# adelowo/cap

Hardware: AMD Instinct MI355X
Metric: verified JWTs/sec (RS256-2048, ES256) at 1/2/4/8 MI355X vs all-core Go CPU (higher is better)
Workload: dtype u32 (28-bit limbs, 64-bit v_mad_u64_u32 accumulators); 1 GPU; ES256 P-256 JWKS with 4 kids, 1M tokens batch-verified per MI355X (BASELINE configs[1]); kids=4, p256_key_comb_w=26, parallelism=independent shards x1

## Files before the change

### cap_amd/csrc/jg_runtime.cpp

```cpp
#include <pthread.h>
#include <hip/hip_runtime.h>
#include <sched.h>

#include <algorithm>
#include <array>
#include <atomic>
#include <chrono>
#include <condition_variable>
#include <cstddef>
#include <cstdio>
#include <cstdlib>
#include <cstring>
#include <deque>
#include <functional>
#include <map>
#include <set>
#include <memory>
#include <mutex>
#include <shared_mutex>
#include <string>
#include <thread>
#include <unordered_map>
#include <vector>

// ... 38 lines not shown
    const char* e = std::getenv("CAPJWT_RELEASE_GTABLES");
    return e && std::atoi(e) != 0;
  }();
  return on;
}

double ms_since(std::chrono::steady_clock::time_point t) {
  return std::chrono::duration<double, std::milli>(std::chrono::steady_clock::now() - t).count();
}

bool load_trace() {
  static const bool on = std::getenv("CAPJWT_LOAD_TRACE") != nullptr;
  return on;
}
struct PhaseClock {
  std::chrono::steady_clock::time_point t = std::chrono::steady_clock::now();
  void lap(const char* what) {
    if (!load_trace()) return;
    std::fprintf(stderr, "[capjwt load] %-28s %8.2f ms\n", what, ms_since(t));
    t = std::chrono::steady_clock::now();
  }
};

bool zc_env_enabled() {
  const char* e = std::getenv("CAPJWT_ZC");
  return e && std::atoi(e) != 0;
}
size_t zc_env_max_jobs() {
  const char* e = std::getenv("CAPJWT_ZC_MAX");
  const long long v = e ? std::atoll(e) : 0;
  return v >= 64 ? (size_t)v : (size_t)2 << 20;
}

size_t chunk_jobs() {
  static const size_t n = [] {
    if (const char* e = std::getenv("CAPJWT_CHUNK")) {
      const long v = std::atol(e);
      if (v >= 64) return (size_t)v;
    }
    return (size_t)65536;
  }();
  return n;
}

uint64_t default_table_budget() {
  static const uint64_t b = [] {
    if (const char* e = std::getenv("CAPJWT_TABLE_BUDGET_GB")) {
      const double v = std::atof(e);
      if (v >= 0) return (uint64_t)(v * (double)(1ull << 30));
    }
    return (uint64_t)32 << 30;
  }();
  return b;
}

std::vector<size_t> chunk_cuts(size_t lo, size_t hi, size_t C, size_t first = 4096, bool tail_chunk = true) {
  std::vector<size_t> cut{lo};
  for (size_t ramp = std::min<size_t>(C, first); cut.back() < hi; ramp = std::min(C, 2 * ramp))
    cut.push_back(std::min(hi, cut.back() + ramp));
  const size_t tail = C / 4;
  if (tail_chunk && cut.size() > 2 && tail >= 1024 && cut.back() - cut[cut.size() - 2] > tail)
    cut.insert(cut.end() - 1, cut.back() - tail);
  else if (!tail_chunk && cut.size() > 2 && cut.back() - cut[cut.size() - 2] < C / 8)
    cut.erase(cut.end() - 2);
  return cut;
}

int cls_rows_sig(int c, int l4) {
  switch (c) {
    case CLS_RSA2K: case CLS_RSA3K: return rsa_sig_rows(c);
    case CLS_RSA4K: return rsa_sig_rows_l(l4);
    case CLS_P256: case CLS_P384: case CLS_P521: return EC_S_ROW + 17;
    case CLS_ED25519: return 16;
    default: return 0;
  }
}
int cls_rows_scratch(int c, int l4) {
  switch (c) {
    case CLS_RSA2K: case CLS_RSA3K: return 2 * rsa_limbs(c) + rsa_sig_rows(c);
    case CLS_RSA4K: return 2 * l4 + rsa_sig_rows_l(l4);
    case CLS_P256: case CLS_P384: case CLS_P521: return ec_digit_rows(c) + 2 * ec_limbs(c);
    case CLS_ED25519: return 4 * ED_L;
    default: return 0;
  }
}
constexpr double CLS_COST[NCLS] = {0.01, 4.2, 9.0, 15.5, 1.0, 3.4, 6.6, 1.1};

inline size_t grow_size(size_t n, size_t cap) {
  const size_t want = std::max(n, cap + cap / 2);
  return (want + (size_t(2) << 20) - 1) & ~((size_t(2) << 20) - 1);
}

std::atomic<int> g_grows{0};

struct Grow {
  void* p = nullptr;
  size_t cap = 0;
  void* get(size_t n) {
    if (n == 0) n = 16;
    if (n > cap) {
      if (p) (void)hipFree(p);
      p = nullptr;
      const size_t c = grow_size(n, cap);
      cap = 0;
      g_grows.fetch_add(1, std::memory_order_relaxed);
      HIPCHK(hipMalloc(&p, c));
// ... 331 lines not shown
  bool zc = false;
  bool small_ec = true;
  std::atomic<uint64_t>* small_launches = nullptr;
};

class Helper {
 public:
  explicit Helper(int device) : th_([this, device] { loop(device); }) {}
  ~Helper() {
    {
      std::lock_guard<std::mutex> g(m_);
      stop_ = true;
    }
    cv_.notify_all();
    th_.join();
  }
  void run(std::function<void()> f) {
    std::lock_guard<std::mutex> g(m_);
    job_ = std::move(f);
    busy_ = true;
    cv_.notify_all();
  }
  void wait() {
    std::unique_lock<std::mutex> lk(m_);
    cv_.wait(lk, [&] { return !busy_; });
  }

 private:
  void loop(int device) {
    pthread_setname_np(pthread_self(), "capjwt-plan");
    (void)hipSetDevice(device);
    std::unique_lock<std::mutex> lk(m_);
    while (true) {
      cv_.wait(lk, [&] { return stop_ || job_; });
      if (!job_) break;
      auto f = std::move(job_);
      job_ = nullptr;
      lk.unlock();
      f();
      lk.lock();
      busy_ = false;
      cv_.notify_all();
    }
  }
  std::mutex m_;
  std::condition_variable cv_;
  std::function<void()> job_;
  bool busy_ = false, stop_ = false;
  std::thread th_;
};

struct Device {
  int id = 0;
  Lane lane0;
  Lane lane1;
  hipStream_t kstream = nullptr;
  hipStream_t ustream = nullptr;
  hipStream_t clstream = nullptr;
  std::mutex cl_mu;
  Grow cl_arena, cl_jobs, cl_out, cl_expect;
  uint32_t* gtab[NCLS] = {};
  uint32_t* btab = nullptr;
  std::shared_ptr<SharedTable> tab_ref[NCLS];
  std::mutex mu;
  hipStream_t copy = nullptr;
  Lane lanes[NLANE];
  Slot slots[NSLOT + NZSLOT];
  int next_slot = 0, next_lane = 0, next_zslot = 0;
  double gload[3] = {0, 0, 0};
  int next_res = 0;
  std::thread worker, completer;
  std::unique_ptr<Helper> planner;
  std::mutex qmu;
  std::condition_variable qcv;
  std::deque<Item> q;
  bool stop = false;
  std::mutex cmu;
  std::condition_variable ccv, scv;
  std::deque<Slot*> cq;
  bool cstop = false;
};

}

struct jg_batch {
  jg_ctx* ctx = nullptr;
  Device* dev = nullptr;
  Lane* lane = nullptr;
  std::unique_ptr<Bufs> own;
  Bufs* b = nullptr;
  Plan plan;
  size_t arena_len = 0;
  size_t dslot = 0;
  uint64_t epoch = 0;
  KeyStateP ks_run;
  bool timing = true;
  std::vector<std::string> mark_names;
  std::vector<hipEvent_t> mark_events;
  size_t marks_used = 0;
  std::vector<std::string> tnames;
  std::vector<float> tms;
  ~jg_batch() {
    for (auto e : mark_events) (void)hipEventDestroy(e);
  }
};

// ... 249 lines not shown
    P.sig_rows = std::max(P.sig_rows, cls_rows_sig(c, P.rsa4k_limbs));
    P.scratch_rows = std::max(P.scratch_rows, cls_rows_scratch(c, P.rsa4k_limbs));
    if (c <= CLS_RSA4K) {
      P.pss_off[c] = P.pss_tokens;
      P.pss_tokens += P.ranges[c].end - P.ranges[c].begin;
    }
  }
}

inline std::pair<int64_t, int64_t> pad_range(const PlanScratch& X, size_t b, const Plan& P, size_t RB) {
  if (P.npad == WAVE && X.start[RB] == 0 && b == RB) {
    int64_t any = 0;
    for (int64_t t : X.total) any += t;
    if (any == 0) return {0, WAVE};
  }
  return {X.start[b] + X.total[b], X.start[b] + (X.total[b] + WAVE - 1) / WAVE * WAVE};
}

void plan_fill_host(const KeyState& K, const jg_tok* toks, size_t ntok, const Plan& P, PlanScratch& X, JobDev* jobs,
                    int32_t* perm) {
  const size_t nk = K.keys.size(), NB = nk + 1, RB = nk;
  for (size_t b = 0; b < NB; ++b) {
    const auto r = pad_range(X, b, P, RB);
    const JobDev pad{0, 0, 0, job_pack(b == RB ? 0u : (uint32_t)b, JOB_PAD, 0)};
    for (int64_t p = r.first; p < r.second; ++p) {
      jobs[p] = pad;
      perm[p] = -1;
    }
  }
  std::vector<int64_t> cur = X.start;
  for (size_t i = 0; i < ntok; ++i) {
    const jg_tok& tk = toks[i];
    const int c = X.tcls[i];
    const int64_t p = cur[c == CLS_REJECT ? RB : tk.key_idx]++;
    jobs[p] = JobDev{(uint32_t)tk.off, tk.sig_in_len, (uint32_t)(tk.off + tk.sig_rel_off),
                     job_pack(c == CLS_REJECT ? 0u : tk.key_idx, tk.alg, tk.sig_b64_len)};
    perm[p] = (int32_t)i;
  }
}

void size_scratch(Bufs* B, const Plan& P, size_t arena_bytes) {
  const int64_t npad = P.npad;
  const size_t ntok = std::max<size_t>((size_t)P.ntok, 1);
  B->arena.get(arena_bytes + ARENA_SLACK);
  B->sigw.get(sizeof(uint32_t) * P.sig_rows * npad);
  B->dig.get(sizeof(uint32_t) * DIG_ROWS * npad);
  B->status.get(npad);
  B->siglen.get(sizeof(uint16_t) * npad);
  B->vpad.get(npad);
  B->verdict.get(ntok);
  B->rows.get(sizeof(uint32_t) * (size_t)P.scratch_rows * npad);
  B->pss.get((size_t)std::max<int64_t>(P.pss_tokens, 1) * 2048);
  B->exc.get(sizeof(int32_t) * npad);
  B->exc_cnt.get(sizeof(uint32_t) * NCLS);
}

void upload(Bufs* B, hipStream_t s, const Plan& P, const uint8_t* arena, size_t arena_bytes, const JobDev* jobs,
            const int32_t* perm) {
  size_scratch(B, P, arena_bytes);
  B->jobs.get(sizeof(JobDev) * P.npad);
  B->perm.get(sizeof(int32_t) * P.npad);
  uint8_t* da = (uint8_t*)B->arena.p;
  if (arena_bytes && arena) HIPCHK(hipMemcpyAsync(da, arena, arena_bytes, hipMemcpyHostToDevice, s));
  HIPCHK(hipMemsetAsync(da + arena_bytes, 0, ARENA_SLACK, s));
  HIPCHK(hipMemcpyAsync(B->jobs.p, jobs, sizeof(JobDev) * P.npad, hipMemcpyHostToDevice, s));
  HIPCHK(hipMemcpyAsync(B->perm.p, perm, sizeof(int32_t) * P.npad, hipMemcpyHostToDevice, s));
}

struct PlanBlock {
  size_t cur_off, pad_off, zc_off, toks_off, bytes;
  PlanBlock(size_t nbuckets, size_t n) {
    cur_off = 0;
    pad_off = sizeof(uint64_t) * nbuckets;
    zc_off = pad_off + 2 * sizeof(int64_t) * nbuckets;
    toks_off = (zc_off + 3 * sizeof(uint64_t) * nbuckets + 63) & ~size_t(63);
    bytes = toks_off + sizeof(jg_tok) * std::max<size_t>(n, 1);
  }
};

void mark(jg_batch* b, const char* name) {
  if (!b || !b->timing) return;
  if (b->marks_used == b->mark_events.size()) {
    hipEvent_t e;
    HIPCHK(hipEventCreate(&e));
    b->mark_events.push_back(e);
    b->mark_names.emplace_back();
  }
  HIPCHK(hipEventRecord(b->mark_events[b->marks_used], b->lane->stream));
  b->mark_names[b->marks_used] = name;
  ++b->marks_used;
}

const char* cls_name(int c) {
  static const char* n[NCLS] = {"reject", "rsa2048", "rsa3072", "rsa4096", "p256", "p384", "p521", "ed25519"};
  return n[c];
}

struct MarkCtx {
  jg_batch* b;
  int cls;
};
thread_local MarkCtx g_mark_ctx;

void mark_cb(void* p, const char* kname) {
  MarkCtx* m = (MarkCtx*)p;
  mark(m->b, (std::string(cls_name(m->cls)) + "_" + kname).c_str());
}
// ... 108 lines not shown
  for (int oi = 0; oi < NCLS - 1; ++oi) {
    const int c = order[oi];
    const ClassRange r = P.ranges[c];
    if (r.end <= r.begin) continue;
    hipStream_t s = s0;
    if (conc) {
      s = L->cstream[c];
      HIPCHK(hipStreamWaitEvent(s, L->ev_start, 0));
    } else if (gf) {
      s = gf->cls[c];
      if (!feed) HIPCHK(hipStreamWaitEvent(s, gf->start, 0));
    }
    if (zc) {
      ZcGatherArgs za = gf->gather;
      za.begin = r.begin;
      za.end = r.end;
      launch_zc_gather(za, feed ? gf->feed : s);
      if (feed) {
        HIPCHK(hipEventRecord(gf->fed[c], gf->feed));
        HIPCHK(hipStreamWaitEvent(s, gf->fed[c], 0));
      }
    }
    pa.begin = r.begin;
    pa.end = r.end;
    pa.zrows = cls_rows_sig(c, P.rsa4k_limbs);
    pa.ec_words = (c >= CLS_P256 && c <= CLS_P521) ? ec_sig_words(c) : 0;
    launch_prep(c, P.hash_mask[c], pa, s);
    mark(marks, (std::string(cls_name(c)) + "_prep").c_str());
    if (c <= CLS_RSA4K) {
      RsaArgs ra{};
      ra.jobs = pa.jobs; ra.keys = pa.keys; ra.keyblob = pa.keyblob;
      ra.sigw = pa.sigw; ra.dig = pa.dig;
      const int Lm = c == CLS_RSA4K ? P.rsa4k_limbs : rsa_limbs(c);
      ra.xmw = rows;
      ra.xlr = rows + (size_t)Lm * np;
      ra.yw = rows + (size_t)2 * Lm * np;
      ra.status = pa.status; ra.siglen = pa.siglen; ra.verdict_pad = (uint8_t*)B->vpad.p;
      ra.pss_scratch = (uint8_t*)B->pss.p + P.pss_off[c] * 2048;
      ra.has_pss = P.pss_any[c];
      ra.layouts = c == CLS_RSA4K ? P.rsa4k_layouts : 1;
      ra.npad = np; ra.begin = r.begin; ra.end = r.end;
      launch_rsa(c, ra, s, marker(marks, c));
    } else if (c <= CLS_P521) {
      if (!d->gtab[c]) throw std::runtime_error("curve table missing");
      EcArgs ea{};
      ea.jobs = pa.jobs; ea.keys = pa.keys; ea.keyblob = pa.keyblob;
      ea.sigw = pa.sigw; ea.dig = pa.dig; ea.status = pa.status; ea.verdict_pad = (uint8_t*)B->vpad.p;
      ea.digs = rows;
      ea.u1w = rows + (size_t)ec_digit_rows(c) * np;
      ea.u2w = rows + (size_t)(ec_digit_rows(c) + ec_limbs(c)) * np;
      ea.gtab = d->gtab[c];
      ea.exc_list = (int32_t*)B->exc.p + r.begin;
      ea.exc_count = (uint32_t*)B->exc_cnt.p + c;
      ea.npad = np;
      ea.exc_reset = 1;
      ea.part = EC_FAST;
      width_runs(K, G, P, c, [&](int64_t b, int64_t e, int w) {
        ea.begin = b; ea.end = e; ea.wq = w;
        launch_ec(c, ea, s, marker(marks, c));
        ea.exc_reset = 0;
      });
      EcArgs x = ea;
      x.begin = r.begin;
      x.end = r.end;
      x.part = EC_EXACT;
      if (gf) exact_later.push_back({c, x});
      else launch_ec(c, x, s, marker(marks, c));
    } else {
      if (!d->btab) throw std::runtime_error("Ed25519 base table missing");
      EdArgs ea{};
      ea.jobs = pa.jobs; ea.keys = pa.keys; ea.keyblob = pa.keyblob;
      ea.sigw = pa.sigw; ea.dig = pa.dig; ea.status = pa.status; ea.siglen = pa.siglen;
      ea.verdict_pad = (uint8_t*)B->vpad.p;
      ea.xyz = rows;
      ea.btab = d->btab;
      ea.npad = np;
      width_runs(K, G, P, c, [&](int64_t b, int64_t e, int w) {
        ea.begin = b; ea.end = e; ea.wa = w;
        launch_ed(ea, s, marker(marks, c));
      });
    }
    if (s != s0) G.uses.record(s, conc ? "class stream" : "group lane", c);
    if (conc) {
      HIPCHK(hipEventRecord(L->ev_done[c], s));
      HIPCHK(hipStreamWaitEvent(s0, L->ev_done[c], 0));
    } else if (gf) {
      HIPCHK(hipEventRecord(gf->done[c], s));
      if (s != s0) HIPCHK(hipStreamWaitEvent(s0, gf->done[c], 0));
    }
  }
  for (const auto& [c, x] : exact_later) launch_ec(c, x, s0, Marker{});
  launch_scatter((const int32_t*)B->perm.p, (const uint8_t*)B->vpad.p,
                 verdict_dst ? verdict_dst : (uint8_t*)B->verdict.p, np, s0);
  mark(marks, "scatter");
  HIPCHK(hipGetLastError());
  G.uses.record(s0, gf ? "join lane" : "lane");
}

void collect_times(jg_batch* b) {
  b->tnames.clear();
  b->tms.clear();
  for (size_t i = 1; i < b->marks_used; ++i) {
    float ms = 0;
    if (hipEventElapsedTime(&ms, b->mark_events[i - 1], b->mark_events[i]) == hipSuccess) {
      b->tnames.push_back(b->mark_names[i]);
      b->tms.push_back(ms);
// ... 1189 lines not shown
    it.nchunks = it.cuts.size() - 1;
    t->pending += it.nchunks;
    items.push_back(std::move(it));
  }
  for (size_t k = 0, i = 0; k < nd && i < items.size(); ++k) {
    if (cut[k + 1] <= cut[k]) continue;
    Device* d = ctx->devs[k].get();
    Item& it = items[i++];
    if (it.nchunks == 1 && it.hi - it.lo <= SMALL_SUBMIT) {
      bool idle;
      {
        std::lock_guard<std::mutex> g(d->qmu);
        idle = d->q.empty();
      }
      if (idle) {
        process_item(d, k, it);
        continue;
      }
    }
    {
      std::lock_guard<std::mutex> g(d->qmu);
      d->q.push_back(std::move(it));
    }
    d->qcv.notify_one();
  }
  return t;
}

int wait_ticket(jg_ctx* ctx, const std::shared_ptr<Ticket>& t) {
  std::unique_lock<std::mutex> lk(t->m);
  t->cv.wait(lk, [&] { return t->pending == 0; });
  if (t->rc) ctx->set_err(t->err);
  return t->rc;
}

}

extern "C" {

jg_ctx* jg_create(const int* devices, int ndev) {
  try {
    auto ctx = std::make_unique<jg_ctx>();
    int count = 0;
    HIPCHK(hipGetDeviceCount(&count));
    if (count <= 0) throw std::runtime_error("no HIP device");
    std::vector<int> ids;
    if (!devices || ndev <= 0) ids.push_back(0);
    else ids.assign(devices, devices + ndev);
    for (int id : ids) {
      if (id < 0 || id >= count) throw std::runtime_error("bad device id " + std::to_string(id));
      auto d = std::make_unique<Device>();
      d->id = id;
      HIPCHK(hipSetDevice(id));
      HIPCHK(hipStreamCreateWithFlags(&d->copy, hipStreamNonBlocking));
      for (auto& l : d->lanes) l.create_main();
      d->lane0.create_main();
      d->lane1.create_main();
      d->lane0.create_fanout(RES_GROUP, RES_NGROUPS);
      d->lane1.create_fanout(RES_GROUP, RES_NGROUPS);
      for (auto& s : d->slots) {
        HIPCHK(hipEventCreateWithFlags(&s.done, pipe_trace() ? hipEventDefault : hipEventDisableTiming));
        HIPCHK(hipEventCreateWithFlags(&s.copied, hipEventDisableTiming));
        HIPCHK(hipEventCreate(&s.tr_a));
        HIPCHK(hipEventCreate(&s.tr_b));
        HIPCHK(hipEventCreate(&s.tr_c));
        HIPCHK(hipEventCreateWithFlags(&s.ev_planned, hipEventDisableTiming));
        for (auto& e : s.ev_cls) HIPCHK(hipEventCreateWithFlags(&e, hipEventDisableTiming));
        for (auto& e : s.ev_fed) HIPCHK(hipEventCreateWithFlags(&e, hipEventDisableTiming));
      }
      HIPCHK(hipStreamCreateWithFlags(&d->kstream, hipStreamNonBlocking));
      HIPCHK(hipStreamCreateWithFlags(&d->ustream, hipStreamNonBlocking));
      HIPCHK(hipStreamCreateWithFlags(&d->clstream, hipStreamNonBlocking));
      ctx->devs.push_back(std::move(d));
    }
    auto ks = std::make_shared<KeyState>();
    for (size_t i = 0; i < ctx->devs.size(); ++i) ks->dev.push_back(std::make_shared<DevGen>());
    ctx->ks = ks;
    jg_ctx* c = ctx.release();
    for (size_t i = 0; i < c->devs.size(); ++i) {
      c->devs[i]->planner = std::make_unique<Helper>(c->devs[i]->id);
      c->devs[i]->worker = std::thread(worker_loop, c->devs[i].get(), i);
      c->devs[i]->completer = std::thread(completer_loop, c->devs[i].get());
    }
    c->upgrader = std::thread(upgrade_loop, c);
    return c;
  } catch (const std::exception& e) {
    g_tls_err = e.what();
    return nullptr;
  }
}

void jg_destroy(jg_ctx* ctx) {
  if (!ctx) return;
  {
    std::lock_guard<std::mutex> g(ctx->up_mu);
    ctx->up_stop = true;
  }
  ctx->up_cv.notify_all();
  if (ctx->upgrader.joinable()) ctx->upgrader.join();
  for (auto& d : ctx->devs) {
    {
      std::lock_guard<std::mutex> g(d->qmu);
      d->stop = true;
    }
    d->qcv.notify_all();
    if (d->worker.joinable()) d->worker.join();
// ... 507 lines not shown
```

### cap_amd/csrc/kernels/ecdsa.hpp

```cpp
#pragma once
#include <hip/hip_runtime.h>
#include <cstdint>

#include "common.hpp"
#include "prep.hpp"

struct EcArgs {
  const jgk::JobDev* jobs;
  const jgk::DevKey* keys;
  const uint32_t* keyblob;
  const uint32_t* sigw;
  const uint32_t* dig;
  uint8_t* status;
  uint8_t* verdict_pad;
  uint32_t* digs;
  uint32_t* u1w;
  uint32_t* u2w;
  const uint32_t* gtab;
  int32_t* exc_list;
  uint32_t* exc_count;
  int64_t npad, begin, end;
  int32_t wq;
  int32_t exc_reset;
  int32_t part;
};
enum : int32_t { EC_ALL = 0, EC_FAST = 1, EC_EXACT = 2 };

constexpr int ec_limbs(int cls) { return cls == jgk::CLS_P256 ? 10 : cls == jgk::CLS_P384 ? 15 : 20; }
constexpr int ec_sig_words(int cls) { return cls == jgk::CLS_P256 ? 8 : cls == jgk::CLS_P384 ? 12 : 17; }
#ifndef JG_EC_PACK64
#define JG_EC_PACK64 1
#endif
constexpr bool ec_packed(int cls) { return JG_EC_PACK64 && cls == jgk::CLS_P256; }
constexpr int ec_stride(int cls) { return ec_packed(cls) ? 16 : (2 * ec_limbs(cls) + 3) & ~3; }
constexpr int ec_order_bits(int cls) { return cls == jgk::CLS_P256 ? 256 : cls == jgk::CLS_P384 ? 384 : 521; }
constexpr int ec_comb_w(int cls, bool gen) {
  return cls == jgk::CLS_P256 ? (gen ? 26 : 20) : cls == jgk::CLS_P384 ? (gen ? 24 : 16) : (gen ? 20 : 16);
}
constexpr int ec_windows_w(int cls, int w) { return (ec_order_bits(cls) + 2 + w - 1) / w; }
constexpr int ec_entries(int cls, bool gen) { return 1 << (ec_comb_w(cls, gen) - 1); }
constexpr int ec_windows(int cls, bool gen) { return ec_windows_w(cls, ec_comb_w(cls, gen)); }
constexpr int ec_digit_rows(int cls) { return ec_windows(cls, true) + ec_windows(cls, false); }
constexpr int ec_max_keys(int cls) { return 256; }
constexpr int64_t ec_table_words_w(int cls, int w) {
  return (int64_t)ec_windows_w(cls, w) * (1 << (w - 1)) * ec_stride(cls);
}
constexpr int64_t ec_table_words(int cls, bool gen) { return ec_table_words_w(cls, ec_comb_w(cls, gen)); }
constexpr int EC_P256_WQ[4] = {26, 24, 22, 20};
constexpr int EC_P384_WQ[4] = {24, 20, 18, 16};
constexpr int EC_P521_WQ[3] = {20, 18, 16};
constexpr bool ec_top_window_ok(int cls, int w) { return ec_order_bits(cls) - w * (ec_windows_w(cls, w) - 1) <= w - 2; }
static_assert(ec_top_window_ok(jgk::CLS_P256, 26) && ec_top_window_ok(jgk::CLS_P256, 24) &&
              ec_top_window_ok(jgk::CLS_P256, 22) && ec_top_window_ok(jgk::CLS_P256, 20) &&
              ec_top_window_ok(jgk::CLS_P384, 24) && ec_top_window_ok(jgk::CLS_P384, 20) &&
              ec_top_window_ok(jgk::CLS_P384, 18) && ec_top_window_ok(jgk::CLS_P384, 16) &&
              ec_top_window_ok(jgk::CLS_P521, 20) && ec_top_window_ok(jgk::CLS_P521, 18) &&
              ec_top_window_ok(jgk::CLS_P521, 16), "comb window count leaves no room for the top carry");

void launch_ec(int cls, const EcArgs& a, hipStream_t s, const jgk::Marker& mk);

constexpr int EC_SMALL_MAX = jgk::SMALL_MAX;
constexpr uint32_t EC_SMALL_IN_MAX = jgk::SMALL_IN_MAX;
struct EcSmallArgs {
  const uint8_t* arena;
  const jgk::DevKey* keys;
  const uint32_t* keyblob;
  const uint32_t* gtab;
  uint8_t* verdict;
  uint32_t n;
  jgk::JobDev jobs[EC_SMALL_MAX];
  uint16_t out[EC_SMALL_MAX];
};
void launch_ec_small(int cls, int wq, const EcSmallArgs& a, hipStream_t s);
void launch_ec_keyprep(int cls, jgk::DevKey* keys, uint32_t* blob, const int32_t* idx, int n, hipStream_t s);
void launch_ec_keytables(int cls, int wq, jgk::DevKey* keys, uint32_t* blob, const int32_t* tidx, int tn,
                         hipStream_t s, bool sliced = false);
void launch_ec_gtable(int cls, uint32_t* tab, hipStream_t s);
```

### cap_amd/csrc/kernels/ecdsa_impl.hpp

```cpp
#pragma once
#include <hip/hip_runtime.h>

#include <algorithm>
#include <cstdlib>
#include <type_traits>

#include "common.hpp"
#include "ecdsa.hpp"
#include "inv_shape.hpp"
#include "mp.hpp"
#include "tables.hpp"

using namespace jgk;

namespace {

template <int WQ_>
struct CurveP256W { using Fp = P256P; using Fn = P256N; using C = P256C; static constexpr int CLS = CLS_P256, WQ = WQ_; };
using CurveP256 = CurveP256W<20>;
template <int WQ_>
struct CurveP384W { using Fp = P384P; using Fn = P384N; using C = P384C; static constexpr int CLS = CLS_P384, WQ = WQ_; };
using CurveP384 = CurveP384W<16>;
template <int WQ_>
struct CurveP521W { using Fp = P521P; using Fn = P521N; using C = P521C; static constexpr int CLS = CLS_P521, WQ = WQ_; };
// ... 130 lines not shown
  for (int q = 0; q < EW; ++q) {
    const int src = hw - 1 - q;
    R.ew[q] = src >= 0 ? a.dig[(int64_t)(src < 0 ? 0 : src) * np + p] : 0u;
  }
}

template <class CV>
__device__ __forceinline__ void ec_scalar_re(const EcArgs& a, int64_t p, uint32_t* r, uint32_t* e) {
  using Fn = typename CV::Fn;
  constexpr int L = Fn::L;
  ScalarRaw2<CV> R;
  ec_scalar_load2<CV>(a, p, -1, R);
  mp::words_to_limbs<L, ScalarRaw<CV>::CW>(r, R.rw);
  mp::words_to_limbs<L, ScalarRaw<CV>::EW>(e, R.ew);
  mp::csub<Fn>(e);
}

template <class CV, int W, int NWIN>
__device__ __forceinline__ void store_digit_rows(const EcArgs& a, int64_t p, const uint32_t* u, int row0) {
  constexpr int L = CV::Fn::L;
  constexpr uint32_t DM = (1u << W) - 1u;
  int c = 0;
#pragma unroll
  for (int w = 0; w < NWIN; ++w) {
    const int bit = W * w, q = bit / MP_W, sh = bit % MP_W;
    uint32_t b = q < L ? (u[q] >> sh) : 0u;
    if (sh > MP_W - W && q + 1 < L) b |= u[q + 1] << (MP_W - sh);
    int v = (int)(b & DM) + c;
    c = v >= (1 << (W - 1));
    v -= c << W;
    a.digs[(int64_t)(row0 + w) * a.npad + p] = (uint32_t)v;
  }
}

#ifndef JG_EC_SCALAR_WPB
#define JG_EC_SCALAR_WPB 4
#endif
#ifndef JG_EC_SCALAR_PF
#define JG_EC_SCALAR_PF 0
#endif
constexpr int EC_SCALAR_WPB = JG_EC_SCALAR_WPB;
template <class CV, int WPB = EC_SCALAR_WPB>
#ifndef JG_EC_SCALAR_ATTR
#define JG_EC_SCALAR_ATTR
#endif
__global__ void __launch_bounds__(64 * WPB) JG_EC_SCALAR_ATTR k_ec_scalar_batch(EcArgs a, int B) {
  using Fn = typename CV::Fn;
  constexpr int L = Fn::L;
  const int64_t np = a.npad;
  const int64_t n = a.end - a.begin;
  const int64_t S = (n + B - 1) / B;
  const int64_t i = (int64_t)blockIdx.x * blockDim.x + threadIdx.x;
  if (a.exc_reset && i == 0) *a.exc_count = 0u;
  if (WPB == 1 && i >= S) return;
  uint32_t acc[L];
  mp::set_const<Fn>(acc, Fn::ONE);
  int nb = 0;
  constexpr int WG = ec_comb_w(CV::CLS, true), NG = ec_windows(CV::CLS, true);
  constexpr int WQ = CV::WQ, NQ = ec_windows_w(CV::CLS, CV::WQ);
#if JG_EC_SCALAR_PF
  {
    ScalarRaw<CV> cur, nxt;
    int64_t p = a.begin + i;
    bool have = B > 0 && i < S && p < a.end;
    if (have) ec_scalar_load<CV>(a, p, cur);
    for (int j = 0; have; ++j) {
      const int64_t pn = p + S;
      const bool more = j + 1 < B && pn < a.end;
      if (more) ec_scalar_load<CV>(a, pn, nxt);
      uint32_t r[L], s[L], e[L], sm[L];
      const bool ok = ec_scalar_finish<CV>(a, p, cur, r, s, e);
      if (!ok && job_live(cur.jb)) a.status[p] = ST_REJECT;
      mp::to_mont<Fn>(sm, s);
      mp::mul<Fn>(acc, acc, sm);
#pragma unroll
      for (int k = 0; k < L; ++k) {
        a.u1w[(int64_t)k * np + p] = acc[k];
        a.u2w[(int64_t)k * np + p] = sm[k];
      }
      ++nb;
      if (!more) break;
      cur = nxt;
      p = pn;
    }
  }
  uint32_t inv[L];
  mp::block_inv<Fn, WPB>(inv, acc);
  if (nb > 0) {
    ScalarRaw2<CV> cur, nxt;
    int64_t p = a.begin + i + (int64_t)(nb - 1) * S;
    ec_scalar_load2<CV>(a, p, nb > 1 ? p - S : -1, cur);
    for (int j = nb - 1; j >= 0; --j) {
      if (j > 0) ec_scalar_load2<CV>(a, p - S, j > 1 ? p - 2 * S : -1, nxt);
      uint32_t w[L], r[L], e[L], u1[L], u2[L];
      mp::mul<Fn>(w, inv, cur.cprev);
      mp::mul<Fn>(inv, inv, cur.sm);
      mp::words_to_limbs<L, ScalarRaw<CV>::CW>(r, cur.rw);
      mp::words_to_limbs<L, ScalarRaw<CV>::EW>(e, cur.ew);
      mp::csub<Fn>(e);
      mp::mul<Fn>(u1, e, w); mp::csub<Fn>(u1);
      mp::mul<Fn>(u2, r, w); mp::csub<Fn>(u2);
      store_digit_rows<CV, WG, NG>(a, p, u1, 0);
      store_digit_rows<CV, WQ, NQ>(a, p, u2, NG);
      if (j == 0) break;
      cur = nxt;
      p -= S;
// ... 198 lines not shown
  const int ad = d < 0 ? -d : d;
  const uint32_t* ent = tab + ((int64_t)w * NE + (ad - 1)) * STRIDE;
  uint32_t x2[L], y2[L];
  load_entry<CV>(ent, x2, y2);
  if (d < 0) mp::neg<Fp>(y2, y2);
  if (empty) {
    mp::copy<Fp>(X, x2);
    mp::copy<Fp>(Y, y2); mp::freduce<Fp>(Y);
    mp::set_const<Fp>(Z, Fp::ONE);
    empty = false;
  } else if constexpr (Z1ONE) {
    madd_z1<Fp>(X, Y, Z, x2, y2);
  } else {
    madd<Fp>(X, Y, Z, x2, y2);
  }
}

template <class CV>
__device__ __forceinline__ void load_raw(const uint32_t* __restrict__ ent, uint4* r) {
  const uint4* e4 = reinterpret_cast<const uint4*>(ent);
#pragma unroll
  for (int i = 0; i < 4; ++i) r[i] = e4[i];
}
template <class CV, bool Z1ONE = false>
__device__ __forceinline__ void add_raw(uint32_t* X, uint32_t* Y, uint32_t* Z, bool& empty, const uint4* r, int d) {
  using Fp = typename CV::Fp;
  constexpr int L = Fp::L;
  if (d == 0) return;
  const uint32_t wx[8] = {r[0].x, r[0].y, r[0].z, r[0].w, r[1].x, r[1].y, r[1].z, r[1].w};
  const uint32_t wy[8] = {r[2].x, r[2].y, r[2].z, r[2].w, r[3].x, r[3].y, r[3].z, r[3].w};
  uint32_t x2[L], y2[L];
  mp::words_to_limbs<L, 8>(x2, wx);
  mp::words_to_limbs<L, 8>(y2, wy);
  if (d < 0) mp::neg<Fp>(y2, y2);
  if (empty) {
    mp::copy<Fp>(X, x2);
    mp::copy<Fp>(Y, y2); mp::freduce<Fp>(Y);
    mp::set_const<Fp>(Z, Fp::ONE);
    empty = false;
  } else if constexpr (Z1ONE) {
    madd_z1<Fp>(X, Y, Z, x2, y2);
  } else {
    madd<Fp>(X, Y, Z, x2, y2);
  }
}
#ifndef JG_EC_POINT_PF
#define JG_EC_POINT_PF 0
#endif

#ifndef JG_EC_POINT_ATTR
#define JG_EC_POINT_ATTR
#endif
template <class CV>
__global__ void __launch_bounds__(64) JG_EC_POINT_ATTR k_ec_point(EcArgs a) {
  using Fp = typename CV::Fp;
  using Fn = typename CV::Fn;
  constexpr int L = Fp::L;
  constexpr int NG = ec_windows(CV::CLS, true), NQ = ec_windows_w(CV::CLS, CV::WQ);
  constexpr int NWIN = NG > NQ ? NG : NQ;
  const int64_t p = a.begin + (int64_t)blockIdx.x * WAVE + threadIdx.x;
  const int64_t np = a.npad;
  const JobDev jb = a.jobs[p];
  if (!job_live(jb)) return;
  if (a.status[p] != ST_OK) { a.verdict_pad[p] = 0; return; }
  const int kidx = __builtin_amdgcn_readfirstlane(job_key(jb));
  const uint32_t* __restrict__ qtab = key_table(a.keys[kidx]);
  const uint32_t* __restrict__ gtab = a.gtab;

  uint32_t X[L], Y[L], Z[L];
  bool empty = true;
#if JG_EC_POINT_PF
  if constexpr (ec_packed(CV::CLS) && NG == NQ) {
    constexpr int NS = 2 * NG, STRIDE = ec_stride(CV::CLS);
    constexpr int NEG = ec_entries(CV::CLS, true), NEQ = 1 << (CV::WQ - 1);
    auto dig = [&](int k) { return (int)a.digs[(int64_t)((k & 1) ? NG + (k >> 1) : (k >> 1)) * np + p]; };
    auto ent = [&](int k, int d) {
      const int ad = d < 0 ? -d : d;
      const int64_t idx = ad == 0 ? 0 : ad - 1;
      return (k & 1) ? qtab + ((int64_t)(k >> 1) * NEQ + idx) * STRIDE : gtab + ((int64_t)(k >> 1) * NEG + idx) * STRIDE;
    };
    uint4 rc[4], rn[4];
    int dc = dig(0), dn = dig(1);
    load_raw<CV>(ent(0, dc), rc);
    load_raw<CV>(ent(1, dn), rn);
    int dnn = dig(2);
    add_raw<CV>(X, Y, Z, empty, rc, dc);
#pragma unroll
    for (int i = 0; i < 4; ++i) rc[i] = rn[i];
    dc = dn; dn = dnn;
    load_raw<CV>(ent(2, dn), rn);
    dnn = dig(3);
    add_raw<CV, true>(X, Y, Z, empty, rc, dc);
    for (int k = 2; k < NS; ++k) {
#pragma unroll
      for (int i = 0; i < 4; ++i) rc[i] = rn[i];
      dc = dn; dn = dnn;
      if (k + 1 < NS) load_raw<CV>(ent(k + 1, dn), rn);
      if (k + 2 < NS) dnn = dig(k + 2);
      add_raw<CV>(X, Y, Z, empty, rc, dc);
    }
  } else
#endif
  {
  add_window<CV, true>(X, Y, Z, empty, gtab, 0, (int)a.digs[p]);
  add_window<CV, false, true>(X, Y, Z, empty, qtab, 0, (int)a.digs[(int64_t)NG * np + p]);
  for (int w = 1; w < NWIN; ++w) {
    if (w < NG) add_window<CV, true>(X, Y, Z, empty, gtab, w, (int)a.digs[(int64_t)w * np + p]);
    if (w < NQ) add_window<CV, false>(X, Y, Z, empty, qtab, w, (int)a.digs[(int64_t)(NG + w) * np + p]);
  }
  }
  if (empty) { a.verdict_pad[p] = 0; return; }
  uint32_t zc[L];
  mp::copy<Fp>(zc, Z);
  mp::canon<Fp>(zc);
  if (mp::is_zero_canon<Fp>(zc)) {
    const uint32_t idx = atomicAdd(a.exc_count, 1u);
    a.exc_list[idx] = (int32_t)p;
    a.status[p] = ST_EXCEPTIONAL;
    return;
  }
  constexpr int CW = ec_sig_words(CV::CLS);
  uint32_t rw[CW], r[L];
#pragma unroll
  for (int q = 0; q < CW; ++q) rw[q] = a.sigw[(int64_t)q * np + p];
  mp::words_to_limbs<L, CW>(r, rw);
  uint32_t zz[L], rm[L], tt[L];
  mp::sqr<Fp>(zz, Z);
  mp::to_mont<Fp>(rm, r);
  mp::mul<Fp>(tt, rm, zz);
  bool ok = mp::eq_mod<Fp>(X, tt);
  if (!ok) {
    uint32_t rn[L], pl[L];
    mp::add<Fp>(rn, r, Fn::M);
    mp::norm<Fp>(rn);
    mp::set_const<Fp>(pl, Fp::M);
    if (lt_limbs<L>(rn, pl)) {
      mp::to_mont<Fp>(rm, rn);
      mp::mul<Fp>(tt, rm, zz);
      ok = mp::eq_mod<Fp>(X, tt);
    }
  }
  a.verdict_pad[p] = ok;
}

template <class Fp>
struct JPt { uint32_t X[Fp::L], Y[Fp::L], Z[Fp::L]; bool inf; };

template <class Fp>
__device__ bool is_zero_mod(const uint32_t* a) {
  uint32_t c[Fp::L];
  mp::copy<Fp>(c, a);
  mp::canon<Fp>(c);
  return mp::is_zero_canon<Fp>(c);
}

template <class Fp>
__device__ void times2(uint32_t* r, const uint32_t* a) {
  mp::add<Fp>(r, a, a);
  mp::freduce<Fp>(r);
}

template <class CV>
__device__ void jdbl(JPt<typename CV::Fp>& R, const JPt<typename CV::Fp>& P) {
  using Fp = typename CV::Fp;
  constexpr int L = Fp::L;
  if (P.inf || is_zero_mod<Fp>(P.Y)) { R.inf = true; return; }
  uint32_t delta[L], gamma[L], beta[L], t1[L], t2[L], alpha[L], b2[L], b4[L], b8[L], x3[L], y3[L], z3[L];
  mp::sqr<Fp>(delta, P.Z);
  mp::sqr<Fp>(gamma, P.Y);
  mp::mul<Fp>(beta, P.X, gamma);
  mp::sub<Fp>(t1, P.X, delta);
  mp::add<Fp>(t2, P.X, delta);
  mp::mul<Fp>(alpha, t1, t2);
  uint32_t three[L];
  mp::set_const<Fp>(three, CV::C::THREE_M);
  mp::mul<Fp>(alpha, alpha, three);
  times2<Fp>(b2, beta); times2<Fp>(b4, b2); times2<Fp>(b8, b4);
  mp::sqr<Fp>(x3, alpha);
  mp::sub<Fp>(x3, x3, b8); mp::freduce<Fp>(x3);
  mp::mul<Fp>(z3, P.Y, P.Z);
  times2<Fp>(z3, z3);
  mp::sub<Fp>(t1, b4, x3);
  mp::mul<Fp>(y3, alpha, t1);
  mp::sqr<Fp>(t2, gamma);
  times2<Fp>(t2, t2); times2<Fp>(t2, t2); times2<Fp>(t2, t2);
  mp::sub<Fp>(y3, y3, t2); mp::freduce<Fp>(y3);
  mp::copy<Fp>(R.X, x3); mp::copy<Fp>(R.Y, y3); mp::copy<Fp>(R.Z, z3);
  R.inf = false;
}

template <class CV>
__device__ void jadd(JPt<typename CV::Fp>& R, const JPt<typename CV::Fp>& P, const JPt<typename CV::Fp>& Q) {
  using Fp = typename CV::Fp;
  constexpr int L = Fp::L;
  if (P.inf) { R = Q; return; }
// ... 360 lines not shown
}

template <class CV>
__global__ void k_ec_table_g(uint32_t* tab) {
  constexpr int W = ec_comb_w(CV::CLS, true), NWIN = ec_windows(CV::CLS, true);
  constexpr int NE = ec_entries(CV::CLS, true), STRIDE = ec_stride(CV::CLS);
  const int e = blockIdx.x * blockDim.x + threadIdx.x;
  if (e >= NWIN * NE || e % NE == 0) return;
  table_entry<CV, W>(tab + (int64_t)e * STRIDE, tab + (int64_t)(e / NE) * NE * STRIDE, e % NE + 1);
}

#ifndef JG_EC_SPLIT
#define JG_EC_SPLIT 4
#endif
#ifndef JG_EC_SCALAR_SOLO_MAX
#define JG_EC_SCALAR_SOLO_MAX 16384
#endif
constexpr int64_t EC_SCALAR_SOLO_MAX = JG_EC_SCALAR_SOLO_MAX;
#ifndef JG_EC_SPLIT_MAX
#define JG_EC_SPLIT_MAX 16384
#endif
#ifndef JG_EC_SPLIT2_P256
#define JG_EC_SPLIT2_P256 131072
#endif
constexpr int64_t EC_SPLIT2_MAX_P256 = JG_EC_SPLIT2_P256;
#ifndef JG_EC_PF_MAX
#define JG_EC_PF_MAX 262144
#endif
constexpr int64_t EC_PF_MAX_TOKENS = JG_EC_PF_MAX;
#ifndef JG_EC_SPLIT_PF
#define JG_EC_SPLIT_PF 0
#endif
constexpr int EC_SPLIT = JG_EC_SPLIT;
constexpr int64_t EC_SPLIT_MAX_TOKENS = JG_EC_SPLIT_MAX;

template <class CV>
void launch_chain(const EcArgs& a, hipStream_t s, const Marker& mk) {
  const int64_t waves = (a.end - a.begin) / WAVE;
  dim3 g((unsigned)waves), b(WAVE);
  if (a.part == EC_EXACT) {
    hipLaunchKernelGGL(k_ec_exact<CV>, dim3(64), b, 0, s, a);
    mk("exact");
    return;
  }
  const int64_t n = a.end - a.begin;
  const InvShape sh = inv_shape(n, EC_SCALAR_WPB, EC_SCALAR_SOLO_MAX);
  if (sh.wpb == 1) {
    hipLaunchKernelGGL((k_ec_scalar_batch<CV, 1>), dim3(sh.grid), dim3(WAVE), 0, s, a, sh.B);
  } else {
    hipLaunchKernelGGL(k_ec_scalar_batch<CV>, dim3(sh.grid), dim3(WAVE * EC_SCALAR_WPB), 0, s, a, sh.B);
  }
  mk("scalar");
  bool launched = false;
  if (n <= EC_SPLIT_MAX_TOKENS) {
    hipLaunchKernelGGL((k_ec_point_split<CV, EC_SPLIT, JG_EC_SPLIT_PF != 0>),
                       dim3((unsigned)((n * EC_SPLIT + WAVE - 1) / WAVE)), b, 0, s, a);
    launched = true;
  }
  if constexpr (CV::CLS == jgk::CLS_P256 && EC_SPLIT2_MAX_P256 > 0) {
    if (!launched && n <= EC_SPLIT2_MAX_P256) {
      if (n <= EC_PF_MAX_TOKENS)
        hipLaunchKernelGGL((k_ec_point_split<CV, 2, true>), dim3((unsigned)((n * 2 + WAVE - 1) / WAVE)), b, 0, s, a);
      else
        hipLaunchKernelGGL((k_ec_point_split<CV, 2>), dim3((unsigned)((n * 2 + WAVE - 1) / WAVE)), b, 0, s, a);
      launched = true;
    }
  }
  constexpr int64_t pf_max = CV::CLS == jgk::CLS_P521 ? std::min<int64_t>(EC_PF_MAX_TOKENS, 65536) : EC_PF_MAX_TOKENS;
  if (!launched && n <= pf_max) {
    hipLaunchKernelGGL((k_ec_point_split<CV, 1, true>), dim3((unsigned)((n + WAVE - 1) / WAVE)), b, 0, s, a);
    launched = true;
  }
  if (!launched) hipLaunchKernelGGL(k_ec_point<CV>, g, b, 0, s, a);
  mk("point");
  if (a.part == EC_FAST) return;
  hipLaunchKernelGGL(k_ec_exact<CV>, dim3(64), b, 0, s, a);
  mk("exact");
}

template <class CV>
void keyprep_chain(DevKey* keys, uint32_t* blob, const int32_t* idx, int n, hipStream_t s) {
  if (n > 0) hipLaunchKernelGGL(k_ec_keyprep<CV>, dim3((n + 63) / 64), dim3(64), 0, s, keys, blob, idx, n);
}

template <class CV>
void keytables_chain(DevKey* keys, uint32_t* blob, const int32_t* tidx, int tn, hipStream_t s, bool sliced) {
  constexpr int NWIN = ec_windows_w(CV::CLS, CV::WQ), NE = 1 << (CV::WQ - 1);
  if (tn <= 0) return;
  dim3 b(64);
  hipLaunchKernelGGL(k_ec_table_base_keys<CV>, dim3((NWIN + 63) / 64, tn), b, 0, s, keys, blob, tidx, tn);
  table_slices(NWIN * NE, tn, sliced, s, [&](int e0, int e1, dim3 g) {
    hipLaunchKernelGGL(k_ec_table_keys<CV>, g, b, 0, s, keys, blob, tidx, tn, e0, e1);
  });
}

template <class CV>
void gtable_chain(uint32_t* tab, hipStream_t s) {
  constexpr int NWIN = ec_windows(CV::CLS, true), NE = ec_entries(CV::CLS, true);
  hipLaunchKernelGGL(k_ec_table_base_g<CV>, dim3((NWIN + 63) / 64), dim3(64), 0, s, tab);
  hipLaunchKernelGGL(k_ec_table_g<CV>, dim3((NWIN * NE + 63) / 64), dim3(64), 0, s, tab);
}

}
```

Measured before the change: 660.8 million verified JWTs/s.

## Make P-256 point kernel persistent with atomic wave-group work stealing

Turns the generic ECDSA point kernel for P-256 into a persistent kernel. It launches about JG_EC_POINT_SLOTS blocks per SIMD, and each wave pulls 64-token groups from a global atomic counter until the batch is exhausted. The counter is reset in the scalar-batch kernel and stored next to the exception counters. Debug environment variables can force this path and override the block count. The goal is to cut block scheduling overhead and tail imbalance on large batches, at the cost of one atomic per group and possibly lower occupancy if the slot count is too small. With the default chunk of 65536 and split thresholds, the path may only run for large chunks, so whether it is active is uncertain.

```diff
diff --git a/cap_amd/csrc/jg_runtime.cpp b/cap_amd/csrc/jg_runtime.cpp
--- a/cap_amd/csrc/jg_runtime.cpp
+++ b/cap_amd/csrc/jg_runtime.cpp
@@ -114,6 +114,27 @@
     return (uint64_t)32 << 30;
   }();
   return b;
+}
+
+bool ec_force_point() {
+  static const bool on = [] {
+    const char* e = std::getenv("CAPJWT_DEBUG_EC_POINT");
+    return e && std::atoi(e) != 0;
+  }();
+  return on;
+}
+int ec_point_blocks_env() {
+  static const int n = [] {
+    const char* e = std::getenv("CAPJWT_DEBUG_EC_POINT_BLOCKS");
+    const long v = e ? std::atol(e) : 0;
+    return v >= 1 && v <= (1 << 24) ? (int)v : 0;
+  }();
+  return n;
+}
+int ec_point_blocks(int simds, int cls) {
+  if (!ec_point_persistent(cls)) return 0;
+  if (const int n = ec_point_blocks_env()) return n;
+  return JG_EC_POINT_SLOTS * simds;
 }
 
 std::vector<size_t> chunk_cuts(size_t lo, size_t hi, size_t C, size_t first = 4096, bool tail_chunk = true) {
@@ -551,6 +572,7 @@
 
 struct Device {
   int id = 0;
+  int simds = 0;
   Lane lane0;
   Lane lane1;
   hipStream_t kstream = nullptr;
@@ -906,7 +928,7 @@
   B->rows.get(sizeof(uint32_t) * (size_t)P.scratch_rows * npad);
   B->pss.get((size_t)std::max<int64_t>(P.pss_tokens, 1) * 2048);
   B->exc.get(sizeof(int32_t) * npad);
-  B->exc_cnt.get(sizeof(uint32_t) * NCLS);
+  B->exc_cnt.get(sizeof(uint32_t) * NCLS * 2);
 }
 
 void upload(Bufs* B, hipStream_t s, const Plan& P, const uint8_t* arena, size_t arena_bytes, const JobDev* jobs,
@@ -1121,6 +1143,10 @@
       ea.gtab = d->gtab[c];
       ea.exc_list = (int32_t*)B->exc.p + r.begin;
       ea.exc_count = (uint32_t*)B->exc_cnt.p + c;
+      ea.grp_next = (uint32_t*)B->exc_cnt.p + NCLS + c;
+      ea.point_blocks = ec_point_blocks(d->simds, c);
+      ea.force_point = ec_force_point();
+      ea.point_exact = ec_point_persistent(c) && ec_point_blocks_env() != 0;
       ea.npad = np;
       ea.exc_reset = 1;
       ea.part = EC_FAST;
@@ -2416,6 +2442,9 @@
       auto d = std::make_unique<Device>();
       d->id = id;
       HIPCHK(hipSetDevice(id));
+      int cus = 0;
+      HIPCHK(hipDeviceGetAttribute(&cus, hipDeviceAttributeMultiprocessorCount, id));
+      d->simds = cus * 4;
       HIPCHK(hipStreamCreateWithFlags(&d->copy, hipStreamNonBlocking));
       for (auto& l : d->lanes) l.create_main();
       d->lane0.create_main();
diff --git a/cap_amd/csrc/kernels/ecdsa.hpp b/cap_amd/csrc/kernels/ecdsa.hpp
--- a/cap_amd/csrc/kernels/ecdsa.hpp
+++ b/cap_amd/csrc/kernels/ecdsa.hpp
@@ -23,8 +23,17 @@
   int32_t wq;
   int32_t exc_reset;
   int32_t part;
+  uint32_t* grp_next;
+  int32_t point_blocks;
+  int32_t force_point;
+  int32_t point_exact;
 };
 enum : int32_t { EC_ALL = 0, EC_FAST = 1, EC_EXACT = 2 };
+
+#ifndef JG_EC_POINT_SLOTS
+#define JG_EC_POINT_SLOTS 4
+#endif
+constexpr bool ec_point_persistent(int cls) { return cls == jgk::CLS_P256; }
 
 constexpr int ec_limbs(int cls) { return cls == jgk::CLS_P256 ? 10 : cls == jgk::CLS_P384 ? 15 : 20; }
 constexpr int ec_sig_words(int cls) { return cls == jgk::CLS_P256 ? 8 : cls == jgk::CLS_P384 ? 12 : 17; }
diff --git a/cap_amd/csrc/kernels/ecdsa_impl.hpp b/cap_amd/csrc/kernels/ecdsa_impl.hpp
--- a/cap_amd/csrc/kernels/ecdsa_impl.hpp
+++ b/cap_amd/csrc/kernels/ecdsa_impl.hpp
@@ -206,6 +206,7 @@
   const int64_t S = (n + B - 1) / B;
   const int64_t i = (int64_t)blockIdx.x * blockDim.x + threadIdx.x;
   if (a.exc_reset && i == 0) *a.exc_count = 0u;
+  if (a.grp_next && i == 0) *a.grp_next = 0u;
   if (WPB == 1 && i >= S) return;
   uint32_t acc[L];
   mp::set_const<Fn>(acc, Fn::ONE);
@@ -510,13 +511,12 @@
 #define JG_EC_POINT_ATTR
 #endif
 template <class CV>
-__global__ void __launch_bounds__(64) JG_EC_POINT_ATTR k_ec_point(EcArgs a) {
+__device__ __forceinline__ void ec_point_token(const EcArgs& a, const int64_t p) {
   using Fp = typename CV::Fp;
   using Fn = typename CV::Fn;
   constexpr int L = Fp::L;
   constexpr int NG = ec_windows(CV::CLS, true), NQ = ec_windows_w(CV::CLS, CV::WQ);
   constexpr int NWIN = NG > NQ ? NG : NQ;
-  const int64_t p = a.begin + (int64_t)blockIdx.x * WAVE + threadIdx.x;
   const int64_t np = a.npad;
   const JobDev jb = a.jobs[p];
   if (!job_live(jb)) return;
@@ -599,6 +599,22 @@
     }
   }
   a.verdict_pad[p] = ok;
+}
+
+template <class CV>
+__global__ void __launch_bounds__(64) JG_EC_POINT_ATTR k_ec_point(EcArgs a) {
+  if constexpr (!ec_point_persistent(CV::CLS)) {
+    ec_point_token<CV>(a, a.begin + (int64_t)blockIdx.x * WAVE + threadIdx.x);
+    return;
+  }
+  const uint32_t groups = (uint32_t)((a.end - a.begin) / WAVE);
+  for (;;) {
+    uint32_t g = 0;
+    if (threadIdx.x == 0) g = atomicAdd(a.grp_next, 1u);
+    g = __builtin_amdgcn_readfirstlane(g);
+    if (g >= groups) return;
+    ec_point_token<CV>(a, a.begin + (int64_t)g * WAVE + threadIdx.x);
+  }
 }
 
 template <class Fp>
@@ -1065,13 +1081,14 @@
   }
   mk("scalar");
   bool launched = false;
-  if (n <= EC_SPLIT_MAX_TOKENS) {
+  const bool small_ok = a.force_point == 0;
+  if (small_ok && n <= EC_SPLIT_MAX_TOKENS) {
     hipLaunchKernelGGL((k_ec_point_split<CV, EC_SPLIT, JG_EC_SPLIT_PF != 0>),
                        dim3((unsigned)((n * EC_SPLIT + WAVE - 1) / WAVE)), b, 0, s, a);
     launched = true;
   }
   if constexpr (CV::CLS == jgk::CLS_P256 && EC_SPLIT2_MAX_P256 > 0) {
-    if (!launched && n <= EC_SPLIT2_MAX_P256) {
+    if (small_ok && !launched && n <= EC_SPLIT2_MAX_P256) {
       if (n <= EC_PF_MAX_TOKENS)
         hipLaunchKernelGGL((k_ec_point_split<CV, 2, true>), dim3((unsigned)((n * 2 + WAVE - 1) / WAVE)), b, 0, s, a);
       else
@@ -1080,11 +1097,17 @@
     }
   }
   constexpr int64_t pf_max = CV::CLS == jgk::CLS_P521 ? std::min<int64_t>(EC_PF_MAX_TOKENS, 65536) : EC_PF_MAX_TOKENS;
-  if (!launched && n <= pf_max) {
+  if (small_ok && !launched && n <= pf_max) {
     hipLaunchKernelGGL((k_ec_point_split<CV, 1, true>), dim3((unsigned)((n + WAVE - 1) / WAVE)), b, 0, s, a);
     launched = true;
   }
-  if (!launched) hipLaunchKernelGGL(k_ec_point<CV>, g, b, 0, s, a);
+  if (!launched) {
+    if constexpr (ec_point_persistent(CV::CLS)) {
+      if (a.point_exact) g.x = (unsigned)a.point_blocks;
+      else if (a.point_blocks > 0) g.x = (unsigned)std::min<int64_t>(waves, a.point_blocks);
+    }
+    hipLaunchKernelGGL(k_ec_point<CV>, g, b, 0, s, a);
+  }
   mk("point");
   if (a.part == EC_FAST) return;
   hipLaunchKernelGGL(k_ec_exact<CV>, dim3(64), b, 0, s, a);
```

Measured after the change: 676.8 million verified JWTs/s (median of 6 runs). 2.4% higher.
